# scottberry/TmLibrary

Measured on AMD Instinct MI355X. Metric: sites/sec (2160×2560 uint16) illumstats+correct; % of HBM roofline at 1–8 GPUs, higher is better.
Workload: dtype f64 stats / f32 correct (±1 DN)

## Files before the change

tmlibrary_amd/csrc/abi_apply.hip:

```cpp
#include <cmath>
#include <cstdlib>
#include <map>
#include <mutex>

#include "abi_internal.h"

namespace tmh {

static std::vector<double> gaussian_taps(double sigma) {
  const int lw = (int)(4.0 * sigma + 0.5);
  std::vector<double> w(2 * lw + 1, 0.0);
  w[lw] = 1.0;
  double sum = 1.0;
  const double sd2 = sigma * sigma;
  for (int ii = 1; ii <= lw; ++ii) {
    const double t = std::exp(-0.5 * (double)(ii * ii) / sd2);
    w[lw + ii] = t;
    w[lw - ii] = t;
    sum += 2.0 * t;
  }
  for (auto& x : w) x /= sum;
  return w;
}

// ... 109 lines not shown
    launch_build_corr_lut(c->lut.p, c->log_transform, zero_log10, c->stream);
    corrector_init(c, dev_mean, dev_std);
  } catch (...) {
    delete c;
    throw;
  }
  *out = c;
}

}

extern "C" {

int tmh_smooth_f64_device(const double* dev_in, double* dev_out, double* dev_tmp, int height,
                          int width, double sigma, void* stream) {
  return guard([&] { smooth_dev(dev_in, dev_out, dev_tmp, height, width, sigma, stream); });
}

int tmh_smooth2_f64_device(const double* dev_in0, const double* dev_in1, double* dev_out0,
                           double* dev_out1, double* dev_tmp0, double* dev_tmp1, int height,
                           int width, double sigma, void* stream) {
  return guard([&] {
    TMH_CHECK(dev_in0 && dev_in1 && dev_out0 && dev_out1 && dev_tmp0 && dev_tmp1 && height > 0 &&
                  width > 0,
              TMH_EINVAL, "bad arguments");
    TMH_CHECK(sigma >= 0.125, TMH_EINVAL, "sigma must be >= 0.125");
    const double* ins[2] = {dev_in0, dev_in1};
    const double* outs[2] = {dev_out0, dev_out1};
    for (const double* t : {(const double*)dev_tmp0, (const double*)dev_tmp1})
      for (int k = 0; k < 2; ++k)
        TMH_CHECK(t != ins[k] && t != outs[k], TMH_EINVAL, "dev_tmp0/1 must be buffers of their own");
    TMH_CHECK(dev_tmp0 != dev_tmp1, TMH_EINVAL, "dev_tmp0 and dev_tmp1 must differ");
    TMH_CHECK(dev_out0 != dev_out1, TMH_EINVAL, "dev_out0 and dev_out1 must differ");
    const auto t = taps_for(sigma);
    launch_smooth2(dev_in0, dev_in1, dev_out0, dev_out1, dev_tmp0, dev_tmp1, height, width,
                   t.first, t.second, (hipStream_t)stream);
  });
}

int tmh_smooth_f64(const double* host_in, double* host_out, int height, int width, double sigma) {
  return guard([&] {
    TMH_CHECK(host_in && host_out && height > 0 && width > 0, TMH_EINVAL, "bad arguments");
    const size_t npx = (size_t)height * width;
    DBuf<double> a, b, t;
    a.upload(host_in, npx);
    b.alloc(npx);
    t.alloc(npx);
    smooth_dev(a.p, b.p, t.p, height, width, sigma, nullptr);
    TMH_HIP(hipDeviceSynchronize());
    b.download(host_out, npx);
  });
}

int tmh_corrector_create_device(const double* dev_mean, const double* dev_std, int height,
                                int width, int log_transform, double zero_log10, void* stream,
                                tmh_corrector** out) {
  return guard([&] {
    corrector_create_dev(dev_mean, dev_std, height, width, log_transform, zero_log10, stream, out);
  });
}

int tmh_corrector_create(const double* host_mean, const double* host_std, int height, int width,
                         int log_transform, double zero_log10, tmh_corrector** out) {
  return guard([&] {
    TMH_CHECK(out && host_mean && host_std && height > 0 && width > 0, TMH_EINVAL, "bad arguments");
    const size_t npx = (size_t)height * width;
    DBuf<double> m, s;
    m.upload(host_mean, npx);
    s.upload(host_std, npx);
    corrector_create_dev(m.p, s.p, height, width, log_transform, zero_log10, nullptr, out);
    TMH_HIP(hipDeviceSynchronize());
  });
}

void tmh_corrector_destroy(tmh_corrector* c) {
  if (!c) return;
  (void)hipStreamSynchronize(c->stream);
  if (c->ev_tail) {
    (void)hipEventSynchronize(c->ev_tail);
    (void)hipEventDestroy(c->ev_tail);
  }
  delete c;
}

int tmh_corrector_set_option(tmh_corrector* c, int option, int value) {
  return guard([&] {
    TMH_CHECK(c, TMH_EINVAL, "corrector is NULL");
    if (option == TMH_OPT_FUSED_BANDS) {
      TMH_CHECK(value == 0 || value == 8 || value == 16 || value == 32 || value == 64, TMH_EINVAL,
                "fused bands must be 0 (automatic), 8, 16, 32 or 64");
      c->bands = value;
      return;
    }
    if (option == TMH_OPT_FUSED_CUS) {
      int cus = 256;
      TMH_HIP(hipDeviceGetAttribute(&cus, hipDeviceAttributeMultiprocessorCount, c->device));
      TMH_CHECK(value >= 0 && value <= cus, TMH_EINVAL, "fused CUs must be 0..CU count");
      c->n_wg = value ? value : cus;
      return;
    }
    if (!c->host.set(option, value)) throw Error{TMH_EINVAL, "unknown corrector option"};
  });
}

int tmh_corrector_update_device(tmh_corrector* c, const double* dev_mean, const double* dev_std,
                                void* stream) {
  return guard([&] {
    TMH_CHECK(c && dev_mean && dev_std, TMH_EINVAL, "bad arguments");
    corrector_coeffs(c, dev_mean, dev_std, pick(c->stream, stream));
  });
}

int tmh_corrector_update_multi_device(tmh_corrector* const* cs, int n, const double* const* dev_mean,
                                      const double* const* dev_std, void* stream) {
  return guard([&] {
    TMH_CHECK(cs && dev_mean && dev_std && n >= 1 && n <= kMaxJobs, TMH_EINVAL,
              "bad arguments (1 <= n <= 8 correctors)");
    CoefJobs J{};
    for (int k = 0; k < n; ++k) {
      TMH_CHECK(cs[k] && dev_mean[k] && dev_std[k], TMH_EINVAL, "bad arguments");
      TMH_CHECK(cs[k]->npx == cs[0]->npx, TMH_EINVAL, "correctors of different image sizes");
      coef_job(J, k, cs[k], dev_mean[k], dev_std[k]);
    }
    for (int k = 0; k < n; ++k)
      TMH_CHECK(cs[k]->H == cs[0]->H && cs[k]->W == cs[0]->W, TMH_EINVAL,
                "correctors of different image shapes");
    const hipStream_t s = pick(cs[0]->stream, stream);
    ProfScope prof("coeffs", s);
    launch_coeffs_jobs(J, n, cs[0]->H, cs[0]->W, false, s);
  });
}

int tmh_job_planes_multi_device(tmh_stats* const* hs, tmh_corrector* const* cs, int n,
                                double* const* dev_mean, double* const* dev_std,
                                double* const* dev_smean, double* const* dev_sstd, double sigma,
                                void* stream) {
  return guard([&] {
    TMH_CHECK(hs && cs && dev_smean && dev_sstd && n >= 1 && n <= kMaxJobs, TMH_EINVAL,
              "bad arguments (1 <= n <= 8 jobs)");
    TMH_CHECK(sigma >= 0.125, TMH_EINVAL, "sigma must be >= 0.125");
    for (int k = 0; k < n; ++k) {
      TMH_CHECK(hs[k] && cs[k] && dev_smean[k] && dev_sstd[k], TMH_EINVAL, "bad arguments");
      TMH_CHECK(hs[k]->H == hs[0]->H && hs[k]->W == hs[0]->W && cs[k]->npx == hs[0]->npx,
                TMH_EINVAL, "jobs of different image sizes");
      TMH_CHECK(cs[k]->H == hs[0]->H && cs[k]->W == hs[0]->W, TMH_EINVAL,
                "jobs of different image shapes");
      TMH_CHECK(dev_smean[k] != dev_sstd[k], TMH_EINVAL, "smoothed planes must differ");
      for (int j = 0; j < k; ++j)
        TMH_CHECK(hs[j] != hs[k] && cs[j] != cs[k], TMH_EINVAL, "a handle listed twice");
    }
    const int H = hs[0]->H, W = hs[0]->W;
    const int64_t npx = hs[0]->npx;
    const hipStream_t s = pick(hs[0]->stream, stream);
    for (int k = 0; k < n; ++k) cross_begin(hs[k], s);
    for (int k = 0; k < n; ++k) {
      const bool m = dev_mean && dev_mean[k], d = dev_std && dev_std[k];
      if (m || d)
        launch_finalize(hs[k]->mean.p, hs[k]->m2.p, hs[k]->n, npx, m ? dev_mean[k] : nullptr,
                        d ? dev_std[k] : nullptr, s);
    }
    const auto t = taps_for(sigma);
    const double* in[kMaxPlanes];
    double* out[kMaxPlanes];
    double sq[kMaxPlanes];
    DBuf<double> scratch;
    const bool onepass = t.second == 20 && W >= 41 && !getenv("TMH_SMOOTH_2PASS");
    if (!onepass) scratch.alloc((size_t)3 * n * npx);
    double* tmp[kMaxPlanes];
    for (int k = 0; k < n; ++k) {
      tmh_stats* h = hs[k];
      in[2 * k] = h->mean.p;
      out[2 * k] = dev_smean[k];
      sq[2 * k] = 0.0;
      out[2 * k + 1] = dev_sstd[k];
      if (onepass) {
        in[2 * k + 1] = h->m2.p;
        sq[2 * k + 1] = h->n >= 2 ? (double)(h->n - 1) : -1.0;
      } else {
        double* sd = scratch.p + (size_t)(3 * k) * npx;
        launch_finalize(h->mean.p, h->m2.p, h->n, npx, nullptr, sd, s);
        in[2 * k + 1] = sd;
        sq[2 * k + 1] = 0.0;
        tmp[2 * k] = scratch.p + (size_t)(3 * k + 1) * npx;
        tmp[2 * k + 1] = scratch.p + (size_t)(3 * k + 2) * npx;
      }
    }
    const int nt = coef_tiles(H, W);
    double* psum[kMaxPlanes];
    double* pmin[kMaxPlanes];
    for (int k = 0; k < n; ++k) {
      psum[2 * k] = cs[k]->partial.p + nt;
      pmin[2 * k] = nullptr;
      psum[2 * k + 1] = cs[k]->partial.p;
      pmin[2 * k + 1] = cs[k]->partial.p + 2 * nt;
    }
    launch_smooth_planes(in, out, onepass ? out : tmp, sq, 2 * n, H, W, t.first, t.second, s,
                         psum, pmin);
    CoefJobs J{};
    for (int k = 0; k < n; ++k) coef_job(J, k, cs[k], dev_smean[k], dev_sstd[k]);
    {
      ProfScope prof("coeffs", s);
      launch_coeffs_jobs(J, n, H, W, true, s);
    }
    for (int k = 0; k < n; ++k) cross_end(hs[k], s);
    if (!onepass) TMH_HIP(hipStreamSynchronize(s));
  });
}

int tmh_corrector_means(tmh_corrector* c, double* mean_of_std, double* mean_of_mean) {
  return guard([&] {
    TMH_CHECK(c, TMH_EINVAL, "corrector is NULL");
    double sums[2];
    TMH_HIP(hipStreamSynchronize(c->stream));
    TMH_HIP(hipMemcpy(sums, c->sums.p, 16, hipMemcpyDeviceToHost));
    if (mean_of_std) *mean_of_std = sums[0] / (double)c->npx;
    if (mean_of_mean) *mean_of_mean = sums[1] / (double)c->npx;
  });
}

int tmh_correct_u16_device(tmh_corrector* c, const uint16_t* dev_in, uint16_t* dev_out,
                           int64_t n_sites, int clip_lo, int clip_hi, void* stream) {
  return guard([&] {
    TMH_CHECK(c && (dev_in && dev_out || n_sites == 0) && n_sites >= 0, TMH_EINVAL, "bad arguments");
    check_clip(clip_lo, clip_hi, 65535);
    hipStream_t s = pick(c->stream, stream);
    const FixList fl = corrector_fixlist(c, n_sites, s);
    corrector_forms(c, s);
    launch_correct_u16(dev_in, dev_out, c->npx, n_sites, c->coef.p, c->lut.p, c->mconst.p, fl,
                       c->log_transform, clip_lo, clip_hi, s);
    launch_fix_correct(dev_in, dev_out, 2, c->npx, n_sites, fl, c->coef64.p, c->rc.p,
                       c->log_transform, clip_lo, clip_hi, s);
  });
}

int tmh_correct_u16(tmh_corrector* c, const uint16_t* host_in, uint16_t* host_out, int64_t n_sites,
                    int clip_lo, int clip_hi) {
  return guard([&] {
    TMH_CHECK(c && (host_in && host_out || n_sites == 0) && n_sites >= 0, TMH_EINVAL,
              "bad arguments");
    check_clip(clip_lo, clip_hi, 65535);
    if (n_sites == 0) return;
    const int64_t step =
        std::max<int64_t>(1, std::min<int64_t>({16, n_sites, ((int64_t)192 << 20) / (c->npx * 2)}));
    const size_t slot_px = (size_t)step * c->npx;
    if (2 * slot_px > c->stage_in.n) {
      TMH_HIP(hipStreamSynchronize(c->stream));
      c->stage_in.ensure(2 * slot_px);
      c->stage_out.ensure(2 * slot_px);
    }
    HostPipe& p = c->pipe;
    p.init();
    const bool pinned_in = c->host.staging == kStagingPinnedIn,
               pinned_out = c->host.staging != kStagingDirect;
    auto retire = [&](int slot) {
      if (!p.busy[slot]) return;
      TMH_HIP(hipEventSynchronize(p.ev_done[slot]));
      if (pinned_out)
        par_copy(host_out + p.s0[slot] * c->npx, p.out[slot].p, (size_t)p.ns[slot] * c->npx * 2,
                 c->host.copy_threads);
      p.busy[slot] = false;
    };
    int64_t k = 0;
    try {
      for (int64_t s0 = 0; s0 < n_sites; s0 += step, ++k) {
        const int slot = (int)(k & 1);
        const int64_t ns = std::min(step, n_sites - s0);
        const size_t bytes = (size_t)ns * c->npx * 2;
        retire(slot);
        const void* src = host_in + s0 * c->npx;
        void* dst = host_out + s0 * c->npx;
        if (pinned_in) {
          p.in[slot].ensure(slot_px * 2);
          par_copy(p.in[slot].p, src, bytes, c->host.copy_threads);
          src = p.in[slot].p;
        }
        if (pinned_out) {
          p.out[slot].ensure(slot_px * 2);
          dst = p.out[slot].p;
        }
        uint16_t* din = c->stage_in.p + (size_t)slot * slot_px;
        uint16_t* dout = c->stage_out.p + (size_t)slot * slot_px;
        TMH_HIP(hipMemcpyAsync(din, src, bytes, hipMemcpyHostToDevice, p.h2d));
        TMH_HIP(hipEventRecord(p.ev_in[slot], p.h2d));
        TMH_HIP(hipStreamWaitEvent(c->stream, p.ev_in[slot], 0));
        const FixList fl = corrector_fixlist(c, ns, c->stream);
        corrector_forms(c, c->stream);
        launch_correct_u16(din, dout, c->npx, ns, c->coef.p, c->lut.p, c->mconst.p, fl,
                           c->log_transform, clip_lo, clip_hi, c->stream);
        launch_fix_correct(din, dout, 2, c->npx, ns, fl, c->coef64.p, c->rc.p, c->log_transform,
                           clip_lo, clip_hi, c->stream);
        TMH_HIP(hipEventRecord(p.ev_kern[slot], c->stream));
        TMH_HIP(hipStreamWaitEvent(p.d2h, p.ev_kern[slot], 0));
        TMH_HIP(hipMemcpyAsync(dst, dout, bytes, hipMemcpyDeviceToHost, p.d2h));
        TMH_HIP(hipEventRecord(p.ev_done[slot], p.d2h));
        p.busy[slot] = true;
        p.s0[slot] = s0;
        p.ns[slot] = ns;
      }
      retire((int)(k & 1));
      retire((int)((k + 1) & 1));
    } catch (...) {
      p.abandon(c->stream);
      throw;
    }
  });
}

// ... 24 lines not shown
```

tmlibrary_amd/csrc/abi_internal.h:

```cpp
#pragma once

#include <algorithm>
#include <vector>

#include "common.h"

#pragma GCC visibility push(hidden)

namespace tmh {

template <typename F>
inline int guard(F&& f) {
  try {
    f();
    return TMH_OK;
  } catch (const Error& e) {
    set_error(e.msg);
    return e.code;
  } catch (const std::bad_alloc&) {
    set_error("host allocation failed");
    return TMH_ENOMEM;
  } catch (...) {
    set_error("unknown error");
    return TMH_EDEVICE;
  }
}

template <typename T>
struct DBuf {
  T* p = nullptr;
  size_t n = 0;
  void alloc(size_t count, bool zero = false) {
    release();
    if (count == 0) return;
    if (hipMalloc(&p, count * sizeof(T)) != hipSuccess) {
      p = nullptr;
      throw Error{TMH_ENOMEM, "hipMalloc of " + std::to_string(count * sizeof(T)) + " bytes failed"};
    }
    n = count;
    if (zero) {
      TMH_HIP(hipMemset(p, 0, count * sizeof(T)));
      TMH_HIP(hipDeviceSynchronize());
    }
  }
  void ensure(size_t count, bool zero = false) {
    if (count > n) alloc(count, zero);
  }
  void upload(const void* host, size_t count) {
    alloc(count);
    TMH_HIP(hipMemcpy(p, host, count * sizeof(T), hipMemcpyHostToDevice));
  }
  void download(void* host, size_t count) const {
    TMH_HIP(hipMemcpy(host, p, count * sizeof(T), hipMemcpyDeviceToHost));
  }
  void release() {
    if (p) (void)hipFree(p);
    p = nullptr;
    n = 0;
  }
  ~DBuf() { release(); }
};

struct PinBuf {
  void* p = nullptr;
  size_t n = 0;
  void ensure(size_t bytes) {
    if (bytes <= n) return;
    release();
    if (hipHostMalloc(&p, bytes, hipHostMallocDefault) != hipSuccess) {
      p = nullptr;
      throw Error{TMH_ENOMEM, "hipHostMalloc of " + std::to_string(bytes) + " bytes failed"};
    }
    n = bytes;
  }
  void release() {
    if (p) (void)hipHostFree(p);
    p = nullptr;
    n = 0;
  }
  ~PinBuf() { release(); }
};

void par_copy(void* dst, const void* src, size_t bytes, int max_t);

constexpr int kStagingDirect = 0, kStagingPinnedIn = 1, kStagingPinnedOut = 2;

struct HostOpts {
  int copy_threads = 8;
  int staging = kStagingPinnedOut;
  bool set(int option, int value) {
    if (option == TMH_OPT_COPY_THREADS) {
      TMH_CHECK(value >= 1 && value <= 64, TMH_EINVAL, "copy threads must be 1..64");
      copy_threads = value;
      return true;
    }
    if (option == TMH_OPT_HOST_STAGING) {
      TMH_CHECK(value >= 0 && value <= 2, TMH_EINVAL, "host staging must be 0, 1 or 2");
      staging = value;
      return true;
    }
    return false;
  }
};

struct HostPipe {
  PinBuf in[2], out[2];
  hipStream_t h2d = nullptr, d2h = nullptr;
  hipEvent_t ev_in[2]{}, ev_kern[2]{}, ev_done[2]{};
  bool busy[2] = {false, false};
  int64_t s0[2] = {0, 0}, ns[2] = {0, 0};
  void init() {
    if (h2d) return;
    TMH_HIP(hipStreamCreateWithFlags(&h2d, hipStreamNonBlocking));
    TMH_HIP(hipStreamCreateWithFlags(&d2h, hipStreamNonBlocking));
    for (int i = 0; i < 2; ++i) {
      TMH_HIP(hipEventCreateWithFlags(&ev_in[i], hipEventDisableTiming));
      TMH_HIP(hipEventCreateWithFlags(&ev_kern[i], hipEventDisableTiming));
      TMH_HIP(hipEventCreateWithFlags(&ev_done[i], hipEventDisableTiming));
    }
  }
  void abandon(hipStream_t compute) {
    if (h2d) (void)hipStreamSynchronize(h2d);
    if (d2h) (void)hipStreamSynchronize(d2h);
    if (compute) (void)hipStreamSynchronize(compute);
    busy[0] = busy[1] = false;
  }
  ~HostPipe() {
    if (!h2d) return;
    (void)hipStreamSynchronize(h2d);
    (void)hipStreamSynchronize(d2h);
    for (int i = 0; i < 2; ++i) {
      (void)hipEventDestroy(ev_in[i]);
      (void)hipEventDestroy(ev_kern[i]);
      (void)hipEventDestroy(ev_done[i]);
    }
    (void)hipStreamDestroy(h2d);
    (void)hipStreamDestroy(d2h);
  }
};

}

using namespace tmh;

struct tmh_stats {
  int device = 0;
  int H = 0, W = 0;
  int64_t npx = 0;
  int Q = 0;
  double scale = 0.0;
  unsigned flags = 0;
  int64_t batch_cap = 0;
  hipStream_t own_stream = nullptr;
  hipStream_t stream = nullptr;
  hipStream_t side = nullptr;
  hipStream_t tail = nullptr;
  hipEvent_t ev_fork = nullptr, ev_join = nullptr;
  hipEvent_t ev_in = nullptr, ev_out = nullptr;
  static constexpr int kJoins = 8;
  hipEvent_t join_ev[kJoins]{};
  hipStream_t join_s[kJoins]{};
  int join_n = 0;
  int fused_cfg = kFusedAuto;
  int wf_parts = 0;
  HostOpts host;
  bool hist_dirty = false;
  int64_t n = 0;
  int64_t n_deferred = 0;
  int64_t last_batch = 0;
  int64_t pending = 0;
  DBuf<unsigned long long> wide;
  DBuf<unsigned int> probe;
  unsigned int* probe_host = nullptr;
  hipEvent_t ev_probe = nullptr;
  bool probed = false;
  bool probe_queued = false;
  unsigned int probe_cnt[3] = {0u, 0u, 0u};
  int64_t wide_sites = 0;
  bool pct_sum_external = false;
  DBuf<double> mean, m2, lut_log, gamma, acc, tmp_mean, tmp_std, rn;
  DBuf<double> wf_part;
  DBuf<int32_t> q_lo, q_hi;
  DBuf<unsigned long long> pooled, pooled_parts;
  DBuf<uint32_t> hist_hi, site_hist, hist_full;
  DBuf<unsigned long long> hist_rmask;
  DBuf<uint16_t> rare_v;
  DBuf<unsigned int> rare_n;
  QPos qp{};
  DBuf<uint16_t> stage;
  HostPipe pipe;
  DBuf<uint32_t> vlh;
  int64_t vlh_cap = 0;
  int64_t vlh_ld = 0;
  DBuf<int64_t> zeros;
};

struct tmh_corrector {
  int device = 0;
  int H = 0, W = 0;
  int64_t npx = 0;
  int log_transform = 1;
  double zero_log10 = -10.0;
  hipStream_t stream = nullptr;
  DBuf<float4> coef, mconst, mconst2;
  DBuf<float2> lut, coef2, coef_lin;
  DBuf<double2> coef64;
  DBuf<RefineConst> rc;
  DBuf<unsigned long long> fix_e;
  DBuf<unsigned int> fix_n;
  DBuf<tmh_window> win;
  DBuf<uint8_t> lut8;
  int n_wg = 256;
  int bands = 0;
  bool forms_stale = false;
  DBuf<int> queues;
  DBuf<double> sums, partial;
  DBuf<uint16_t> stage_in, stage_out;
  DBuf<uint8_t> stage8_in, stage8_out;
  HostPipe pipe;
  HostOpts host;
  hipEvent_t ev_tail = nullptr;
  bool tail_pending = false;
};

namespace tmh {

inline hipStream_t pick(hipStream_t own, void* s) { return s ? (hipStream_t)s : own; }

inline hipStream_t hstream(tmh_stats* h) {
  for (int i = 0; i < h->join_n; ++i) TMH_HIP(hipStreamWaitEvent(h->stream, h->join_ev[i], 0));
  h->join_n = 0;
  return h->stream;
}

inline hipStream_t hpick(tmh_stats* h, void* stream) {
  return stream ? (hipStream_t)stream : hstream(h);
}

void defer_join(tmh_stats* h, hipStream_t s);

inline void cross_begin(tmh_stats* h, hipStream_t s) {
  if (s == h->stream) {
    hstream(h);
    return;
  }
  TMH_HIP(hipEventRecord(h->ev_in, h->stream));
  TMH_HIP(hipStreamWaitEvent(s, h->ev_in, 0));
  for (int i = 0; i < h->join_n; ++i)
    if (h->join_s[i] != s) TMH_HIP(hipStreamWaitEvent(s, h->join_ev[i], 0));
}
inline void cross_end(tmh_stats* h, hipStream_t s) {
  if (s == h->stream) return;
  defer_join(h, s);
}

size_t os_words(const tmh_stats* h, int64_t n_sites);
void stats_reserve_sites(tmh_stats* h, int64_t n_sites);
void stats_grow_deferred(tmh_stats* h, int64_t extra);
void stats_probe(tmh_stats* h, const uint16_t* d, int64_t ns, const SiteTab& tab, hipStream_t s);
int probe_fused_cfg(const tmh_stats* h);
SiteTab blocked_tab(const uint16_t* const* dev_in_blocks, uint16_t* const* dev_out_blocks,
                    int block_shift, int64_t npx);
FixList corrector_fixlist(tmh_corrector* c, int64_t n_sites);
FixList corrector_fixlist(tmh_corrector* c, int64_t n_sites, hipStream_t s);
void corrector_forms(tmh_corrector* c, hipStream_t s);
void check_clip(int lo, int hi, int maxv);

}

#pragma GCC visibility pop
```

tmlibrary_amd/csrc/abi_stats.hip:

```cpp
#include <cstring>

#include "abi_internal.h"

namespace tmh {

void defer_join(tmh_stats* h, hipStream_t s) {
  int i = 0;
  while (i < h->join_n && h->join_s[i] != s) ++i;
  if (i == tmh_stats::kJoins) {
    hstream(h);
    i = 0;
  }
  hipEvent_t& e = h->join_ev[i];
  if (!e) TMH_HIP(hipEventCreateWithFlags(&e, hipEventDisableTiming));
  TMH_HIP(hipEventRecord(e, s));
  h->join_s[i] = s;
  if (i == h->join_n) ++h->join_n;
}

size_t os_words(const tmh_stats* h, int64_t n_sites) {
  return (size_t)n_sites * (size_t)os_tiles(h->Q) * kOsTile;
}

void stats_reserve_sites(tmh_stats* h, int64_t n_sites) {
  const bool grow = (size_t)n_sites * kHiBins > h->hist_hi.n || (size_t)n_sites > h->zeros.n ||
                    ((h->flags & 2u) && (size_t)n_sites * kBins > h->site_hist.n) ||
                    (!(h->flags & TMH_STATS_DEFERRED_PCT) && os_words(h, n_sites) > h->vlh.n);
  if (grow) {
    TMH_HIP(hipStreamSynchronize(hstream(h)));
    TMH_HIP(hipStreamSynchronize(h->side));
  }
  if ((size_t)n_sites * kHiBins > h->hist_hi.n) h->hist_hi.alloc((size_t)n_sites * kHiBins, true);
  h->zeros.ensure((size_t)n_sites);
  if (h->flags & 2u) h->site_hist.ensure((size_t)n_sites * kBins);
  if (!(h->flags & TMH_STATS_DEFERRED_PCT)) {
    h->vlh.ensure(os_words(h, n_sites));
  }
}

void stats_grow_deferred(tmh_stats* h, int64_t extra) {
  const int64_t need = h->n_deferred + extra;
  if (need <= h->vlh_cap) {
    h->vlh_ld = h->vlh_cap;
    return;
  }
  const int64_t cap = std::max(need, 2 * h->vlh_cap);
  DBuf<uint32_t> nb;
  nb.alloc(os_words(h, cap));
  if (h->n_deferred) {
    const size_t row = (size_t)kOsTile * 4;
    TMH_HIP(hipMemcpy2DAsync(nb.p, (size_t)cap * row, h->vlh.p, (size_t)h->vlh_cap * row,
                             (size_t)h->n_deferred * row, (size_t)os_tiles(h->Q),
                             hipMemcpyDeviceToDevice, hstream(h)));
  }
  TMH_HIP(hipStreamSynchronize(hstream(h)));
  TMH_HIP(hipStreamSynchronize(h->side));
  std::swap(h->vlh.p, nb.p);
  std::swap(h->vlh.n, nb.n);
  h->vlh_cap = cap;
  h->vlh_ld = cap;
}

void stats_probe(tmh_stats* h, const uint16_t* d, int64_t ns, const SiteTab& tab, hipStream_t s) {
  if (h->probed || (ns <= 0 && !h->probe_queued)) return;
  if (!h->probe_queued) {
    launch_site_probe(d, h->npx, ns, h->probe.p, s, tab);
    TMH_HIP(hipMemcpyAsync(h->probe_host, h->probe.p, 3 * sizeof(unsigned int),
                           hipMemcpyDeviceToHost, s));
    TMH_HIP(hipEventRecord(h->ev_probe, s));
  }
  TMH_HIP(hipEventSynchronize(h->ev_probe));
  for (int i = 0; i < 3; ++i) h->probe_cnt[i] = h->probe_host[i];
  h->probed = true;
  h->probe_queued = false;
}

static void stats_probe_queue(tmh_stats* h, const uint16_t* d, int64_t ns, const SiteTab& tab,
                              hipStream_t s) {
  if (h->probed || h->probe_queued || ns <= 0) return;
  launch_site_probe(d, h->npx, ns, h->probe.p, s, tab);
  TMH_HIP(hipMemcpyAsync(h->probe_host, h->probe.p, 3 * sizeof(unsigned int),
                         hipMemcpyDeviceToHost, s));
  TMH_HIP(hipEventRecord(h->ev_probe, s));
  h->probe_queued = true;
}

static bool probe_bright(const tmh_stats* h) {
  return h->probed && (double)h->probe_cnt[1] >= kBrightFrac * (double)h->probe_cnt[0];
}
int probe_fused_cfg(const tmh_stats* h) {
  if (h->fused_cfg != kFusedAuto) return h->fused_cfg;
  if (!h->probed) return kFusedNarrow;
  const double g = (double)h->probe_cnt[0];
  if ((double)h->probe_cnt[2] >= kXWideFrac * g) return kFusedNoHist;
  if ((double)h->probe_cnt[1] >= kWideFrac * g) return kFusedWide;
  return kFusedNarrow;
}

static void stats_update_dev(tmh_stats* h, const uint16_t* d, int64_t ns, int log_transform,
                             hipStream_t s) {
  if (ns <= 0) return;
  if ((size_t)ns > h->rn.n) {
    TMH_HIP(hipStreamSynchronize(s));
    h->rn.alloc((size_t)ns);
  }
  const bool serial = (h->flags & TMH_STATS_SERIAL) != 0;
  hipStream_t hs = serial ? s : h->side;
  const int64_t chunk = 4096;
  stats_reserve_sites(h, std::min(chunk, ns));
  if (h->flags & TMH_STATS_DEFERRED_PCT) stats_grow_deferred(h, ns);
  const bool vec = (h->npx & 7) == 0 && (reinterpret_cast<uintptr_t>(d) & 15) == 0;
  if (vec && log_transform && h->wf_parts == 0 && ns >= 96) stats_probe(h, d, ns, SiteTab{}, s);
  if (!serial) {
    TMH_HIP(hipEventRecord(h->ev_fork, s));
    TMH_HIP(hipStreamWaitEvent(hs, h->ev_fork, 0));
  }
  launch_welford(d, h->npx, ns, h->n, h->rn.p, h->mean.p, h->m2.p, h->lut_log.p,
                 log_transform, h->wf_part.p, h->wf_part.n, h->wf_parts, nullptr,
                 probe_bright(h) ? 1 : 0, s);
  for (int64_t c0 = 0; c0 < ns; c0 += chunk) {
    const int64_t nc = std::min(chunk, ns - c0);
    const bool deferred = (h->flags & TMH_STATS_DEFERRED_PCT) != 0;
    uint32_t* vlh = h->vlh.p + (deferred ? (size_t)h->n_deferred * kOsTile : 0);
    const int64_t ld = deferred ? h->vlh_cap : nc;
    launch_hist_scatter(d + c0 * h->npx, h->npx, nc, h->hist_hi.p, h->qp, vlh, ld, h->pooled.p,
                        h->zeros.p, (h->flags & 2u) ? h->site_hist.p : nullptr, hs);
    if (deferred)
      h->n_deferred += nc;
    else
      launch_pct_accumulate(vlh, nc, ld, h->Q, h->gamma.p, h->acc.p, hs);
    h->vlh_ld = ld;
    h->last_batch = nc;
  }
  if (!serial) {
    TMH_HIP(hipEventRecord(h->ev_join, hs));
    TMH_HIP(hipStreamWaitEvent(s, h->ev_join, 0));
  }
  h->n += ns;
}

static void stats_welford_dev(tmh_stats* h, const uint16_t* dev_sites, int64_t n_sites,
                              int log_transform, void* stream, const SiteTab& tab) {
  hipStream_t s = hpick(h, stream);
  cross_begin(h, s);
  if ((size_t)n_sites > h->rn.n) {
    TMH_HIP(hipStreamSynchronize(s));
    h->rn.alloc((size_t)n_sites);
  }
  const bool vec = tab.in || ((h->npx & 7) == 0 && (reinterpret_cast<uintptr_t>(dev_sites) & 15) == 0);
  if (vec && (h->fused_cfg == kFusedAuto || (log_transform && h->wf_parts == 0)))
    stats_probe(h, dev_sites, n_sites, tab, s);
  launch_welford(dev_sites, h->npx, n_sites, h->n, h->rn.p, h->mean.p, h->m2.p, h->lut_log.p,
                 log_transform, h->wf_part.p, h->wf_part.n, h->wf_parts, h->wide.p,
                 probe_bright(h) ? 1 : 0, s, tab);
  if ((h->npx & 7) == 0) h->wide_sites += n_sites;
  h->n += n_sites;
  h->pending += n_sites;
  cross_end(h, s);
}

SiteTab blocked_tab(const uint16_t* const* dev_in_blocks, uint16_t* const* dev_out_blocks,
                    int block_shift, int64_t npx) {
  TMH_CHECK(dev_in_blocks, TMH_EINVAL, "block table is NULL");
  TMH_CHECK(block_shift >= 2 && block_shift <= 24, TMH_EINVAL, "block_shift must be 2..24");
  TMH_CHECK((npx & 7) == 0, TMH_EINVAL,
            "blocked site layouts need height * width divisible by 8 (16-byte pixel groups)");
  SiteTab t;
  t.in = dev_in_blocks;
  t.out = dev_out_blocks;
  t.shift = block_shift;
  return t;
}

static void stats_pct_sum_device(tmh_stats* h) {
  if ((h->flags & TMH_STATS_DEFERRED_PCT) && !h->pct_sum_external) {
    TMH_HIP(hipMemsetAsync(h->acc.p, 0, (size_t)h->Q * 8, hstream(h)));
    launch_pct_accumulate(h->vlh.p, h->n_deferred, h->vlh_cap, h->Q, h->gamma.p, h->acc.p,
                          hstream(h));
  }
}

}

extern "C" {

int tmh_stats_create(int height, int width, int n_quantiles, const int64_t* q_lo,
                     const int64_t* q_hi, const double* q_gamma, const double* lut_log10,
                     int batch_capacity, unsigned flags, tmh_stats** out) {
  return guard([&] {
    TMH_CHECK(out, TMH_EINVAL, "out is NULL");
    TMH_CHECK(height > 0 && width > 0, TMH_EINVAL, "image dimensions must be positive");
    const int64_t npx = (int64_t)height * width;
    TMH_CHECK(npx < (int64_t(1) << 31), TMH_EINVAL, "images must have fewer than 2^31 pixels");
    TMH_CHECK(n_quantiles > 0 && q_lo && q_hi && q_gamma && lut_log10, TMH_EINVAL,
              "quantile tables and LUT are required");
    auto* h = new tmh_stats();
    try {
      TMH_HIP(hipGetDevice(&h->device));
      h->H = height;
      h->W = width;
      h->npx = npx;
      h->Q = n_quantiles;
      h->scale = (npx > 1) ? (double)(n_quantiles - 1) / (double)(npx - 1) : 0.0;
      h->flags = flags;
      h->batch_cap = std::min(4096, batch_capacity > 0 ? batch_capacity : 1);
      TMH_HIP(hipStreamCreateWithFlags(&h->own_stream, hipStreamNonBlocking));
      TMH_HIP(hipStreamCreateWithFlags(&h->side, hipStreamNonBlocking));

      TMH_HIP(hipEventCreateWithFlags(&h->ev_fork, hipEventDisableTiming));
      TMH_HIP(hipEventCreateWithFlags(&h->ev_join, hipEventDisableTiming));
      TMH_HIP(hipEventCreateWithFlags(&h->ev_in, hipEventDisableTiming));
      TMH_HIP(hipEventCreateWithFlags(&h->ev_out, hipEventDisableTiming));
      h->stream = h->own_stream;
      h->mean.alloc(npx, true);
      h->m2.alloc(npx, true);
      h->wf_part.alloc((size_t)8 * npx);
      h->wide.alloc(2, true);
      h->probe.alloc(3);
      TMH_HIP(hipHostMalloc((void**)&h->probe_host, 4 * sizeof(unsigned int), hipHostMallocDefault));
      TMH_HIP(hipEventCreateWithFlags(&h->ev_probe, hipEventDisableTiming));
      h->acc.alloc(n_quantiles, true);
      h->pooled.alloc(kBins, true);
      h->lut_log.alloc(kBins);
      h->gamma.alloc(n_quantiles);
      h->q_lo.alloc(n_quantiles);
      h->q_hi.alloc(n_quantiles);
      std::vector<int32_t> lo(n_quantiles), hi(n_quantiles);
      for (int i = 0; i < n_quantiles; ++i) {
        TMH_CHECK(q_lo[i] >= 0 && q_lo[i] < npx && q_hi[i] >= q_lo[i] && q_hi[i] < npx, TMH_EINVAL,
                  "quantile positions out of range");
        TMH_CHECK(i == 0 || (q_lo[i] >= q_lo[i - 1] && q_hi[i] >= q_hi[i - 1]), TMH_EINVAL,
                  "quantile positions must be non-decreasing");
        lo[i] = (int32_t)q_lo[i];
        hi[i] = (int32_t)q_hi[i];
      }
      TMH_HIP(hipMemcpy(h->q_lo.p, lo.data(), lo.size() * 4, hipMemcpyHostToDevice));
      TMH_HIP(hipMemcpy(h->q_hi.p, hi.data(), hi.size() * 4, hipMemcpyHostToDevice));
      TMH_HIP(hipMemcpy(h->gamma.p, q_gamma, (size_t)n_quantiles * 8, hipMemcpyHostToDevice));
      TMH_HIP(hipMemcpy(h->lut_log.p, lut_log10, (size_t)kBins * 8, hipMemcpyHostToDevice));
      h->pooled_parts.alloc((size_t)kPooledParts * kBins, true);
      h->qp.lo = h->q_lo.p;
      h->qp.hi = h->q_hi.p;
      h->qp.Q = n_quantiles;
      h->qp.scale = h->scale;
      h->qp.last = (int32_t)(npx - 1);
      h->qp.hi_next = 1;
      for (int i = 0; i < n_quantiles; ++i)
        if (hi[i] != std::min<int32_t>(lo[i] + 1, (int32_t)(npx - 1))) h->qp.hi_next = 0;
    } catch (...) {
      tmh_stats_destroy(h);
      throw;
    }
    *out = h;
  });
}

void tmh_stats_destroy(tmh_stats* h) {
  if (!h) return;
  for (int i = 0; i < h->join_n; ++i) (void)hipEventSynchronize(h->join_ev[i]);
  if (h->own_stream) (void)hipStreamSynchronize(h->own_stream);
  if (h->stream && h->stream != h->own_stream) (void)hipStreamSynchronize(h->stream);
  hipStream_t s = h->own_stream, side = h->side, tail = h->tail;
  if (side) (void)hipStreamSynchronize(side);
  if (tail) (void)hipStreamSynchronize(tail);
  if (h->ev_fork) (void)hipEventDestroy(h->ev_fork);
  if (h->ev_join) (void)hipEventDestroy(h->ev_join);
  if (h->ev_in) (void)hipEventDestroy(h->ev_in);
  if (h->ev_out) (void)hipEventDestroy(h->ev_out);
  if (h->ev_probe) (void)hipEventDestroy(h->ev_probe);
  for (hipEvent_t e : h->join_ev)
    if (e) (void)hipEventDestroy(e);
  if (h->probe_host) (void)hipHostFree(h->probe_host);
  delete h;
  if (s) (void)hipStreamDestroy(s);
  if (side) (void)hipStreamDestroy(side);
  if (tail) (void)hipStreamDestroy(tail);
}

int tmh_stats_set_stream(tmh_stats* h, void* stream) {
  return guard([&] {
    TMH_CHECK(h, TMH_EINVAL, "handle is NULL");
    h->stream = stream ? (hipStream_t)stream : h->own_stream;
  });
}

int tmh_stats_set_option(tmh_stats* h, int option, int value) {
  return guard([&] {
    TMH_CHECK(h, TMH_EINVAL, "handle is NULL");
    switch (option) {
      case TMH_OPT_FUSED_CONFIG:
        TMH_CHECK((value >= kFusedAuto && value < kFusedConfigs) || value == kFusedNoHist,
                  TMH_EINVAL, "fused configuration out of range");
        h->fused_cfg = value;
        break;
      case TMH_OPT_WELFORD_PARTS:
        TMH_CHECK(value >= 0 && value <= 4, TMH_EINVAL, "Welford parts must be 0..4");
        h->wf_parts = value;
        break;
      default:
        if (!h->host.set(option, value)) throw Error{TMH_EINVAL, "unknown option"};
    }
  });
}

int tmh_stats_reset(tmh_stats* h) {
  return guard([&] {
    TMH_CHECK(h, TMH_EINVAL, "handle is NULL");
    if (h->hist_dirty) {
      TMH_HIP(hipDeviceSynchronize());
      if (h->hist_full.n)
        TMH_HIP(hipMemsetAsync(h->hist_full.p, 0, h->hist_full.n * 4, hstream(h)));
      if (h->hist_rmask.n)
        TMH_HIP(hipMemsetAsync(h->hist_rmask.p, 0, h->hist_rmask.n * 8, hstream(h)));
      TMH_HIP(hipMemsetAsync(h->pooled_parts.p, 0, h->pooled_parts.n * 8, hstream(h)));
      h->hist_dirty = false;
    }
    ZeroList z;
    z.add(h->mean.p, h->npx);
    z.add(h->m2.p, h->npx);
    z.add(h->acc.p, h->Q);
    z.add(h->pooled.p, kBins);
    z.add(h->wide.p, 2);
    launch_zero_u64(z, hstream(h));
    h->wide_sites = 0;
    h->n = 0;
    h->n_deferred = 0;
    h->last_batch = 0;
    h->pending = 0;
    h->pct_sum_external = false;
    if (h->probe_queued) TMH_HIP(hipEventSynchronize(h->ev_probe));
    h->probed = false;
    h->probe_queued = false;
  });
}

int tmh_stats_probe_device(tmh_stats* h, const uint16_t* dev_sites, int64_t n_sites,
                           void* stream) {
  return guard([&] {
    TMH_CHECK(h && (dev_sites || n_sites == 0) && n_sites >= 0, TMH_EINVAL, "bad arguments");
    if ((h->npx & 7) || (reinterpret_cast<uintptr_t>(dev_sites) & 15)) return;
    stats_probe_queue(h, dev_sites, n_sites, SiteTab{}, hpick(h, stream));
  });
}

int tmh_stats_probe_blocks_device(tmh_stats* h, const uint16_t* const* dev_blocks, int block_shift,
                                  int64_t n_sites, void* stream) {
  return guard([&] {
    TMH_CHECK(h && n_sites >= 0, TMH_EINVAL, "bad arguments");
    const SiteTab tab = blocked_tab(dev_blocks, nullptr, block_shift, h->npx);
    stats_probe_queue(h, nullptr, n_sites, tab, hpick(h, stream));
  });
}

int tmh_stats_update_welford_device(tmh_stats* h, const uint16_t* dev_sites, int64_t n_sites,
                                    int log_transform, void* stream) {
  return guard([&] {
    TMH_CHECK(h && (dev_sites || n_sites == 0) && n_sites >= 0, TMH_EINVAL, "bad arguments");
    stats_welford_dev(h, dev_sites, n_sites, log_transform, stream, SiteTab{});
  });
}

int tmh_stats_update_welford_blocks_device(tmh_stats* h, const uint16_t* const* dev_blocks,
                                           int block_shift, int64_t n_sites, int log_transform,
                                           void* stream) {
  return guard([&] {
    TMH_CHECK(h && n_sites >= 0, TMH_EINVAL, "bad arguments");
    if (n_sites == 0) return;
    stats_welford_dev(h, nullptr, n_sites, log_transform, stream,
                      blocked_tab(dev_blocks, nullptr, block_shift, h->npx));
  });
}

int tmh_stats_update_device(tmh_stats* h, const uint16_t* dev_sites, int64_t n_sites,
                            int log_transform, void* stream) {
  return guard([&] {
    TMH_CHECK(h && (dev_sites || n_sites == 0) && n_sites >= 0, TMH_EINVAL, "bad arguments");
    const hipStream_t s = hpick(h, stream);
    cross_begin(h, s);
    stats_update_dev(h, dev_sites, n_sites, log_transform, s);
    cross_end(h, s);
  });
}

int tmh_stats_zero_counts(tmh_stats* h, int64_t* host_out, int64_t n, void* stream) {
  return guard([&] {
    TMH_CHECK(h && (host_out || n == 0) && n >= 0, TMH_EINVAL, "bad arguments");
    TMH_CHECK(n <= h->last_batch && (size_t)n <= h->zeros.n, TMH_EINVAL,
              "more sites than the last update held");
    if (n == 0) return;
    hipStream_t s = hpick(h, stream);
    cross_begin(h, s);
    TMH_HIP(hipMemcpyAsync(host_out, h->zeros.p, (size_t)n * 8, hipMemcpyDeviceToHost, s));
    cross_end(h, s);
  });
}

int tmh_stats_update(tmh_stats* h, const uint16_t* host_sites, int64_t n_sites, int log_transform,
                     int64_t* zero_counts_out) {
  return guard([&] {
    TMH_CHECK(h && (host_sites || n_sites == 0) && n_sites >= 0, TMH_EINVAL, "bad arguments");
    if (n_sites == 0) return;
    HostPipe& p = h->pipe;
    const int64_t per = h->batch_cap;
    const size_t slot_px = (size_t)per * h->npx;
    if (2 * slot_px > h->stage.n) {
      TMH_HIP(hipStreamSynchronize(hstream(h)));
      h->stage.ensure(2 * slot_px);
    }
    p.init();
    const bool pinned = h->host.staging == kStagingPinnedIn;
    auto retire = [&](int slot) {
      if (!p.busy[slot]) return;
      TMH_HIP(hipEventSynchronize(p.ev_done[slot]));
      if (zero_counts_out)
        std::memcpy(zero_counts_out + p.s0[slot], p.out[slot].p, (size_t)p.ns[slot] * 8);
      p.busy[slot] = false;
    };
    int64_t k = 0;
    try {
      for (int64_t s0 = 0; s0 < n_sites; s0 += per, ++k) {
        const int slot = (int)(k & 1);
        const int64_t ns = std::min<int64_t>(per, n_sites - s0);
        const size_t bytes = (size_t)ns * h->npx * 2;
        retire(slot);
        p.out[slot].ensure((size_t)per * 8);
        const void* src = host_sites + s0 * h->npx;
        if (pinned) {
          p.in[slot].ensure(slot_px * 2);
          par_copy(p.in[slot].p, src, bytes, h->host.copy_threads);
          src = p.in[slot].p;
        }
        uint16_t* dev = h->stage.p + (size_t)slot * slot_px;
        TMH_HIP(hipMemcpyAsync(dev, src, bytes, hipMemcpyHostToDevice, p.h2d));
        TMH_HIP(hipEventRecord(p.ev_in[slot], p.h2d));
        TMH_HIP(hipStreamWaitEvent(hstream(h), p.ev_in[slot], 0));
        stats_update_dev(h, dev, ns, log_transform, hstream(h));
        if (zero_counts_out)
          TMH_HIP(hipMemcpyAsync(p.out[slot].p, h->zeros.p, (size_t)ns * 8, hipMemcpyDeviceToHost,
                                 hstream(h)));
        TMH_HIP(hipEventRecord(p.ev_done[slot], hstream(h)));
        p.busy[slot] = true;
        p.s0[slot] = s0;
        p.ns[slot] = ns;
      }
      retire((int)(k & 1));
      retire((int)((k + 1) & 1));
    } catch (...) {
      p.abandon(hstream(h));
      throw;
    }
  });
}

int tmh_stats_finalize(tmh_stats* h, int64_t* n, double* mean, double* std, double* pct_sum,
                       uint64_t* hist) {
  return guard([&] {
    TMH_CHECK(h, TMH_EINVAL, "handle is NULL");
    if (n) *n = h->n;
    if (mean || std) {
      h->tmp_std.ensure(h->npx);
      launch_finalize(h->mean.p, h->m2.p, h->n, h->npx, nullptr, h->tmp_std.p, hstream(h));
      if (mean)
        TMH_HIP(hipMemcpyAsync(mean, h->mean.p, h->npx * 8, hipMemcpyDeviceToHost, hstream(h)));
      if (std)
        TMH_HIP(hipMemcpyAsync(std, h->tmp_std.p, h->npx * 8, hipMemcpyDeviceToHost, hstream(h)));
    }
    if (pct_sum) {
      stats_pct_sum_device(h);
      TMH_HIP(hipMemcpyAsync(pct_sum, h->acc.p, (size_t)h->Q * 8, hipMemcpyDeviceToHost, hstream(h)));
    }
    if (hist)
      TMH_HIP(hipMemcpyAsync(hist, h->pooled.p, (size_t)kBins * 8, hipMemcpyDeviceToHost, hstream(h)));
    TMH_HIP(hipStreamSynchronize(hstream(h)));
  });
}

int tmh_stats_finalize_device(tmh_stats* h, double* dev_mean, double* dev_std, void* stream) {
  return guard([&] {
    TMH_CHECK(h, TMH_EINVAL, "handle is NULL");
    const hipStream_t s = hpick(h, stream);
    cross_begin(h, s);
    launch_finalize(h->mean.p, h->m2.p, h->n, h->npx, dev_mean, dev_std, s);
    cross_end(h, s);
  });
}

int tmh_stats_variance(tmh_stats* h, double* host_var) {
  return guard([&] {
    TMH_CHECK(h && host_var, TMH_EINVAL, "bad arguments");
    h->tmp_std.ensure(h->npx);
    launch_variance(h->m2.p, h->n, h->npx, h->tmp_std.p, hstream(h));
    TMH_HIP(hipMemcpyAsync(host_var, h->tmp_std.p, h->npx * 8, hipMemcpyDeviceToHost, hstream(h)));
    TMH_HIP(hipStreamSynchronize(hstream(h)));
  });
}

int tmh_stats_job_choice(tmh_stats* h, uint32_t* probe_counts, int* welford_bright,
                         int* fused_cfg) {
  return guard([&] {
    TMH_CHECK(h, TMH_EINVAL, "handle is NULL");
    if (probe_counts)
      for (int i = 0; i < 3; ++i) probe_counts[i] = h->probed ? h->probe_cnt[i] : 0u;
    if (welford_bright) *welford_bright = h->probed ? (probe_bright(h) ? 1 : 0) : -1;
    if (fused_cfg) {
      const int c = probe_fused_cfg(h);
      *fused_cfg = c == kFusedNoHist ? TMH_FUSED_NO_HIST : c;
    }
  });
}

int tmh_stats_wide_groups(tmh_stats* h, uint64_t* groups_out, int64_t* sites_out) {
  return guard([&] {
    TMH_CHECK(h && groups_out, TMH_EINVAL, "bad arguments");
    unsigned long long w = 0;
    TMH_HIP(hipMemcpyAsync(&w, h->wide.p, 8, hipMemcpyDeviceToHost, hstream(h)));
    TMH_HIP(hipStreamSynchronize(hstream(h)));
    *groups_out = w;
    if (sites_out) *sites_out = h->wide_sites;
  });
}

int tmh_stats_get_hist_device(tmh_stats* h, uint64_t* dev_hist, void* stream) {
  return guard([&] {
    TMH_CHECK(h && dev_hist, TMH_EINVAL, "bad arguments");
    const hipStream_t s = hpick(h, stream);
    cross_begin(h, s);
    TMH_HIP(hipMemcpyAsync(dev_hist, h->pooled.p, (size_t)kBins * 8, hipMemcpyDeviceToDevice, s));
    cross_end(h, s);
  });
}

int tmh_stats_set_hist_device(tmh_stats* h, const uint64_t* dev_hist, void* stream) {
  return guard([&] {
    TMH_CHECK(h && dev_hist, TMH_EINVAL, "bad arguments");
    const hipStream_t s = hpick(h, stream);
    cross_begin(h, s);
    TMH_HIP(hipMemcpyAsync(h->pooled.p, dev_hist, (size_t)kBins * 8, hipMemcpyDeviceToDevice, s));
    cross_end(h, s);
  });
}

int tmh_stats_site_histogram(tmh_stats* h, int64_t site, uint32_t* host_hist) {
  return guard([&] {
    TMH_CHECK(h && host_hist, TMH_EINVAL, "bad arguments");
    TMH_CHECK(h->flags & 2u, TMH_ESTATE, "handle was created without TMH_STATS_KEEP_SITE_HIST (2)");
    TMH_CHECK(site >= 0 && site < h->last_batch, TMH_EINVAL, "site outside the last batch");
    TMH_HIP(hipMemcpyAsync(host_hist, h->site_hist.p + (size_t)site * kBins, (size_t)kBins * 4,
                           hipMemcpyDeviceToHost, hstream(h)));
    TMH_HIP(hipStreamSynchronize(hstream(h)));
  });
}

int tmh_stats_site_order_stats(tmh_stats* h, int64_t site, uint16_t* host_vlo, uint16_t* host_vhi) {
  return guard([&] {
    TMH_CHECK(h && host_vlo && host_vhi, TMH_EINVAL, "bad arguments");
    const bool deferred = h->flags & TMH_STATS_DEFERRED_PCT;
    const int64_t avail = deferred ? h->n_deferred : h->last_batch;
    TMH_CHECK(site >= 0 && site < avail, TMH_EINVAL, "site not available");
    const size_t row = (size_t)kOsTile * 4;
    std::vector<uint32_t> w((size_t)os_tiles(h->Q) * kOsTile);
    TMH_HIP(hipMemcpy2DAsync(w.data(), row, h->vlh.p + (size_t)site * kOsTile,
                             (size_t)h->vlh_ld * row, row, (size_t)os_tiles(h->Q),
                             hipMemcpyDeviceToHost, hstream(h)));
    TMH_HIP(hipStreamSynchronize(hstream(h)));
    for (int64_t q = 0; q < h->Q; ++q) {
      host_vlo[q] = (uint16_t)(w[q] & 0xFFFFu);
      host_vhi[q] = (uint16_t)(w[q] >> 16);
    }
    TMH_HIP(hipStreamSynchronize(hstream(h)));
  });
}

int tmh_stats_get_n(tmh_stats* h, int64_t* n) {
  return guard([&] {
    TMH_CHECK(h && n, TMH_EINVAL, "bad arguments");
    *n = h->n;
  });
}

int tmh_stats_set_n(tmh_stats* h, int64_t n) {
  return guard([&] {
    TMH_CHECK(h && n >= 0, TMH_EINVAL, "bad arguments");
    h->n = n;
  });
}

int tmh_stats_merge_stage1(tmh_stats* h, double* dev_nmean, void* stream) {
  return guard([&] {
    TMH_CHECK(h && dev_nmean, TMH_EINVAL, "bad arguments");
    const hipStream_t s = hpick(h, stream);
    cross_begin(h, s);
    launch_merge1(h->mean.p, h->n, h->npx, dev_nmean, s);
    cross_end(h, s);
  });
}

int tmh_stats_merge_stage2(tmh_stats* h, const double* dev_sum_nmean, int64_t n_total,
                           double* dev_m2c, void* stream) {
  return guard([&] {
    TMH_CHECK(h && dev_sum_nmean && dev_m2c && n_total > 0, TMH_EINVAL, "bad arguments");
    const hipStream_t s = hpick(h, stream);
    cross_begin(h, s);
    launch_merge2(h->mean.p, h->m2.p, h->n, dev_sum_nmean, n_total, h->npx, dev_m2c, s);
    cross_end(h, s);
  });
}

int tmh_stats_merge_stage3(tmh_stats* h, int64_t n_total, const double* dev_sum_m2c, void* stream) {
  return guard([&] {
    TMH_CHECK(h && dev_sum_m2c && n_total >= 0, TMH_EINVAL, "bad arguments");
    const hipStream_t s = hpick(h, stream);
    cross_begin(h, s);
    launch_copy_f64(dev_sum_m2c, h->m2.p, h->npx, s);
    cross_end(h, s);
    h->n = n_total;
  });
}

int tmh_stats_pct_accumulate(tmh_stats* h, double* dev_acc, void* stream) {
  return guard([&] {
    TMH_CHECK(h && dev_acc, TMH_EINVAL, "bad arguments");
    TMH_CHECK(h->flags & TMH_STATS_DEFERRED_PCT, TMH_ESTATE,
              "percentile chain needs a TMH_STATS_DEFERRED_PCT handle");
    const hipStream_t s = hpick(h, stream);
    cross_begin(h, s);
    launch_pct_accumulate(h->vlh.p, h->n_deferred, h->vlh_cap, h->Q, h->gamma.p, dev_acc, s);
    cross_end(h, s);
  });
}

int tmh_stats_pct_accumulate_range(tmh_stats* h, double* dev_acc_range, int q_begin, int q_count,
                                   void* stream) {
  return guard([&] {
    TMH_CHECK(h && dev_acc_range, TMH_EINVAL, "bad arguments");
    TMH_CHECK(h->flags & TMH_STATS_DEFERRED_PCT, TMH_ESTATE,
              "percentile chain needs a TMH_STATS_DEFERRED_PCT handle");
    TMH_CHECK(q_begin >= 0 && q_count >= 0 && (int64_t)q_begin + q_count <= h->Q, TMH_EINVAL,
              "quantile range out of bounds");
    const hipStream_t s = hpick(h, stream);
    cross_begin(h, s);
    launch_pct_accumulate_range(h->vlh.p, h->n_deferred, h->vlh_cap, q_begin, q_count, h->gamma.p,
                                dev_acc_range, s);
    cross_end(h, s);
  });
}

int tmh_stats_set_pct_sum(tmh_stats* h, const double* dev_acc, void* stream) {
  return guard([&] {
    TMH_CHECK(h && dev_acc, TMH_EINVAL, "bad arguments");
    const hipStream_t s = hpick(h, stream);
    cross_begin(h, s);
    launch_copy_f64(dev_acc, h->acc.p, h->Q, s);
    cross_end(h, s);
    h->pct_sum_external = true;
  });
}

int tmh_stats_get_pct_sum_device(tmh_stats* h, double* dev_acc, void* stream) {
  return guard([&] {
    TMH_CHECK(h && dev_acc, TMH_EINVAL, "bad arguments");
    hipStream_t s = hpick(h, stream);
    const bool cross = s != h->stream;
    cross_begin(h, s);
    if ((h->flags & TMH_STATS_DEFERRED_PCT) && !h->pct_sum_external) {
      TMH_HIP(hipMemsetAsync(dev_acc, 0, (size_t)h->Q * 8, s));
      launch_pct_accumulate(h->vlh.p, h->n_deferred, h->vlh_cap, h->Q, h->gamma.p, dev_acc, s);
    } else {
      TMH_HIP(hipMemcpyAsync(dev_acc, h->acc.p, (size_t)h->Q * 8, hipMemcpyDeviceToDevice, s));
    }
    if (cross) defer_join(h, s);
  });
}

}
```

Before: 170,700.

## Defer mean/M2 zeroing on reset and map probe counters to pinned host memory

```diff
diff --git a/tmlibrary_amd/csrc/abi_apply.hip b/tmlibrary_amd/csrc/abi_apply.hip
--- a/tmlibrary_amd/csrc/abi_apply.hip
+++ b/tmlibrary_amd/csrc/abi_apply.hip
@@ -285,7 +285,10 @@
     const int H = hs[0]->H, W = hs[0]->W;
     const int64_t npx = hs[0]->npx;
     const hipStream_t s = pick(hs[0]->stream, stream);
-    for (int k = 0; k < n; ++k) cross_begin(hs[k], s);
+    for (int k = 0; k < n; ++k) {
+      cross_begin(hs[k], s);
+      stats_state_fresh(hs[k], s);
+    }
     for (int k = 0; k < n; ++k) {
       const bool m = dev_mean && dev_mean[k], d = dev_std && dev_std[k];
       if (m || d)
diff --git a/tmlibrary_amd/csrc/abi_internal.h b/tmlibrary_amd/csrc/abi_internal.h
--- a/tmlibrary_amd/csrc/abi_internal.h
+++ b/tmlibrary_amd/csrc/abi_internal.h
@@ -165,13 +165,14 @@
   int wf_parts = 0;
   HostOpts host;
   bool hist_dirty = false;
+  bool state_stale = false;
   int64_t n = 0;
   int64_t n_deferred = 0;
   int64_t last_batch = 0;
   int64_t pending = 0;
   DBuf<unsigned long long> wide;
-  DBuf<unsigned int> probe;
   unsigned int* probe_host = nullptr;
+  unsigned int* probe_dev = nullptr;
   hipEvent_t ev_probe = nullptr;
   bool probed = false;
   bool probe_queued = false;
@@ -256,6 +257,7 @@
 
 size_t os_words(const tmh_stats* h, int64_t n_sites);
 void stats_reserve_sites(tmh_stats* h, int64_t n_sites);
+void stats_state_fresh(tmh_stats* h, hipStream_t s);
 void stats_grow_deferred(tmh_stats* h, int64_t extra);
 void stats_probe(tmh_stats* h, const uint16_t* d, int64_t ns, const SiteTab& tab, hipStream_t s);
 int probe_fused_cfg(const tmh_stats* h);
diff --git a/tmlibrary_amd/csrc/abi_stats.hip b/tmlibrary_amd/csrc/abi_stats.hip
--- a/tmlibrary_amd/csrc/abi_stats.hip
+++ b/tmlibrary_amd/csrc/abi_stats.hip
@@ -64,9 +64,7 @@
 void stats_probe(tmh_stats* h, const uint16_t* d, int64_t ns, const SiteTab& tab, hipStream_t s) {
   if (h->probed || (ns <= 0 && !h->probe_queued)) return;
   if (!h->probe_queued) {
-    launch_site_probe(d, h->npx, ns, h->probe.p, s, tab);
-    TMH_HIP(hipMemcpyAsync(h->probe_host, h->probe.p, 3 * sizeof(unsigned int),
-                           hipMemcpyDeviceToHost, s));
+    launch_site_probe(d, h->npx, ns, h->probe_dev, s, tab);
     TMH_HIP(hipEventRecord(h->ev_probe, s));
   }
   TMH_HIP(hipEventSynchronize(h->ev_probe));
@@ -78,11 +76,27 @@
 static void stats_probe_queue(tmh_stats* h, const uint16_t* d, int64_t ns, const SiteTab& tab,
                               hipStream_t s) {
   if (h->probed || h->probe_queued || ns <= 0) return;
-  launch_site_probe(d, h->npx, ns, h->probe.p, s, tab);
-  TMH_HIP(hipMemcpyAsync(h->probe_host, h->probe.p, 3 * sizeof(unsigned int),
-                         hipMemcpyDeviceToHost, s));
+  launch_site_probe(d, h->npx, ns, h->probe_dev, s, tab);
   TMH_HIP(hipEventRecord(h->ev_probe, s));
   h->probe_queued = true;
+}
+
+void stats_state_fresh(tmh_stats* h, hipStream_t s) {
+  if (!h->state_stale) return;
+  ZeroList z;
+  z.add(h->mean.p, h->npx);
+  z.add(h->m2.p, h->npx);
+  launch_zero_u64(z, s);
+  h->state_stale = false;
+}
+
+static void stats_state_welford(tmh_stats* h, const uint16_t* d, int64_t ns, const SiteTab& tab,
+                                hipStream_t s) {
+  const bool vec = tab.in || ((h->npx & 7) == 0 && (reinterpret_cast<uintptr_t>(d) & 15) == 0);
+  if (vec && h->n == 0 && ns > 0)
+    h->state_stale = false;
+  else
+    stats_state_fresh(h, s);
 }
 
 static bool probe_bright(const tmh_stats* h) {
@@ -115,6 +129,7 @@
     TMH_HIP(hipEventRecord(h->ev_fork, s));
     TMH_HIP(hipStreamWaitEvent(hs, h->ev_fork, 0));
   }
+  stats_state_welford(h, d, ns, SiteTab{}, s);
   launch_welford(d, h->npx, ns, h->n, h->rn.p, h->mean.p, h->m2.p, h->lut_log.p,
                  log_transform, h->wf_part.p, h->wf_part.n, h->wf_parts, nullptr,
                  probe_bright(h) ? 1 : 0, s);
@@ -150,6 +165,7 @@
   const bool vec = tab.in || ((h->npx & 7) == 0 && (reinterpret_cast<uintptr_t>(dev_sites) & 15) == 0);
   if (vec && (h->fused_cfg == kFusedAuto || (log_transform && h->wf_parts == 0)))
     stats_probe(h, dev_sites, n_sites, tab, s);
+  stats_state_welford(h, dev_sites, n_sites, tab, s);
   launch_welford(dev_sites, h->npx, n_sites, h->n, h->rn.p, h->mean.p, h->m2.p, h->lut_log.p,
                  log_transform, h->wf_part.p, h->wf_part.n, h->wf_parts, h->wide.p,
                  probe_bright(h) ? 1 : 0, s, tab);
@@ -216,8 +232,8 @@
       h->m2.alloc(npx, true);
       h->wf_part.alloc((size_t)8 * npx);
       h->wide.alloc(2, true);
-      h->probe.alloc(3);
       TMH_HIP(hipHostMalloc((void**)&h->probe_host, 4 * sizeof(unsigned int), hipHostMallocDefault));
+      TMH_HIP(hipHostGetDevicePointer((void**)&h->probe_dev, h->probe_host, 0));
       TMH_HIP(hipEventCreateWithFlags(&h->ev_probe, hipEventDisableTiming));
       h->acc.alloc(n_quantiles, true);
       h->pooled.alloc(kBins, true);
@@ -315,9 +331,8 @@
       TMH_HIP(hipMemsetAsync(h->pooled_parts.p, 0, h->pooled_parts.n * 8, hstream(h)));
       h->hist_dirty = false;
     }
+    h->state_stale = true;
     ZeroList z;
-    z.add(h->mean.p, h->npx);
-    z.add(h->m2.p, h->npx);
     z.add(h->acc.p, h->Q);
     z.add(h->pooled.p, kBins);
     z.add(h->wide.p, 2);
@@ -459,6 +474,7 @@
     if (n) *n = h->n;
     if (mean || std) {
       h->tmp_std.ensure(h->npx);
+      stats_state_fresh(h, hstream(h));
       launch_finalize(h->mean.p, h->m2.p, h->n, h->npx, nullptr, h->tmp_std.p, hstream(h));
       if (mean)
         TMH_HIP(hipMemcpyAsync(mean, h->mean.p, h->npx * 8, hipMemcpyDeviceToHost, hstream(h)));
@@ -480,6 +496,7 @@
     TMH_CHECK(h, TMH_EINVAL, "handle is NULL");
     const hipStream_t s = hpick(h, stream);
     cross_begin(h, s);
+    stats_state_fresh(h, s);
     launch_finalize(h->mean.p, h->m2.p, h->n, h->npx, dev_mean, dev_std, s);
     cross_end(h, s);
   });
@@ -489,6 +506,7 @@
   return guard([&] {
     TMH_CHECK(h && host_var, TMH_EINVAL, "bad arguments");
     h->tmp_std.ensure(h->npx);
+    stats_state_fresh(h, hstream(h));
     launch_variance(h->m2.p, h->n, h->npx, h->tmp_std.p, hstream(h));
     TMH_HIP(hipMemcpyAsync(host_var, h->tmp_std.p, h->npx * 8, hipMemcpyDeviceToHost, hstream(h)));
     TMH_HIP(hipStreamSynchronize(hstream(h)));
@@ -590,6 +608,7 @@
     TMH_CHECK(h && dev_nmean, TMH_EINVAL, "bad arguments");
     const hipStream_t s = hpick(h, stream);
     cross_begin(h, s);
+    stats_state_fresh(h, s);
     launch_merge1(h->mean.p, h->n, h->npx, dev_nmean, s);
     cross_end(h, s);
   });
@@ -601,6 +620,7 @@
     TMH_CHECK(h && dev_sum_nmean && dev_m2c && n_total > 0, TMH_EINVAL, "bad arguments");
     const hipStream_t s = hpick(h, stream);
     cross_begin(h, s);
+    stats_state_fresh(h, s);
     launch_merge2(h->mean.p, h->m2.p, h->n, dev_sum_nmean, n_total, h->npx, dev_m2c, s);
     cross_end(h, s);
   });
@@ -611,6 +631,7 @@
     TMH_CHECK(h && dev_sum_m2c && n_total >= 0, TMH_EINVAL, "bad arguments");
     const hipStream_t s = hpick(h, stream);
     cross_begin(h, s);
+    stats_state_fresh(h, s);
     launch_copy_f64(dev_sum_m2c, h->m2.p, h->npx, s);
     cross_end(h, s);
     h->n = n_total;
```

Result: no change. 171,100 (median of 6 runs) (+0.2%).
